# lukehollis/three-mlagents

Hardware: NVIDIA B200
Metric: env_steps_per_sec (higher is better)
Workload: dtype f32+f64

## Files before the change

### profiles/rollout_ab.py

```python
from __future__ import annotations

import argparse
import json
import os
import shutil
import statistics
import subprocess
import sys
import tempfile

import numpy as np

ROOT = os.path.dirname(os.path.dirname(os.path.abspath(__file__)))


def _run(cmd, cwd):
    r = subprocess.run(cmd, cwd=cwd, capture_output=True, text=True)
    if r.returncode != 0:
        raise RuntimeError(f"{' '.join(cmd)} in {cwd} failed ({r.returncode}):\n{r.stdout[-2000:]}\n{r.stderr[-4000:]}")
    return r.stdout


def _bench(tree, steps, dump=None):
    cmd = [sys.executable, "bench.py", "--quick", "--steps", str(steps)] + (["--dump-outputs", dump] if dump else [])
    return json.loads(_run(cmd, tree).strip().splitlines()[-1])


_TASK_TIMER = """
import sys, torch
sys.path.insert(0, '.')
from three_mlagents_b200.vec_env import CudaVecEnv
task, n, T, K = sys.argv[1], 65536, 128, int(sys.argv[2])
env = CudaVecEnv(task, n, seed=1)
obs = torch.empty((T, n, env.obs_dim), device='cuda')
act = torch.empty((T, n), dtype=torch.int32, device='cuda')
rew = torch.empty((T, n), device='cuda')
done = torch.empty((T, n), dtype=torch.uint8, device='cuda')
for _ in range(50):
    env.rollout_random(T, obs, act, rew, done)
e0, e1 = torch.cuda.Event(enable_timing=True), torch.cuda.Event(enable_timing=True)
e0.record()
for _ in range(K):
    env.rollout_random(T, obs, act, rew, done)
e1.record()
torch.cuda.synchronize()
print(e0.elapsed_time(e1) / K * 1e3)
"""


def _time_task(tree, task, steps):
    return float(_run([sys.executable, "-c", _TASK_TIMER, task, str(steps)], tree).strip().splitlines()[-1])


def _summary(runs, base_name="parent"):
    base = statistics.median(runs[base_name])
    return {name: {"us_per_launch": us, "median_us": statistics.median(us), "spread": (max(us) - min(us)) / statistics.median(us),
                   "gain_vs_parent": 1.0 - statistics.median(us) / base} for name, us in runs.items()}


def main():
    ap = argparse.ArgumentParser()
    ap.add_argument("--parent", required=True, help="untracked export of the parent commit")
    ap.add_argument("--rounds", type=int, default=4)
    ap.add_argument("--steps", type=int, default=200)
    ap.add_argument("--tasks", default="gridworld,push", help="tasks also timed through env.rollout_random ('' for none)")
    ap.add_argument("--out", default=os.path.join(ROOT, "profiles", "rollout_blocks_ab_1gpu.json"))
    args = ap.parse_args()
    trees = {"parent": os.path.abspath(args.parent), "new": ROOT}
    q = "name,power.limit,clocks.max.sm"
    card = _run(["nvidia-smi", f"--query-gpu={q}", "--format=csv,noheader", "-i", "0"], ROOT).strip()
    result = {"card": dict(zip(q.split(","), [c.strip() for c in card.split(",")])),
              "bench": f"bench.py --quick --steps {args.steps}", "rounds": args.rounds}
    for tree in trees.values():
        _run([sys.executable, os.path.join(tree, "three-mlagents_b200", "build.py")], tree)
    tmp = tempfile.mkdtemp(prefix="rollout_ab_")
    try:
        for name, tree in trees.items():
            _bench(tree, 50, dump=os.path.join(tmp, name))
        result["dump_equal"] = {f: bool(np.array_equal(np.load(os.path.join(tmp, "parent", f)), np.load(os.path.join(tmp, "new", f))))
                                for f in ("obs.npy", "actions.npy", "rewards.npy", "dones.npy")}
    finally:
        shutil.rmtree(tmp, ignore_errors=True)
    tasks = [t for t in args.tasks.split(",") if t]
    runs = {name: [] for name in trees}
    task_runs = {task: {name: [] for name in trees} for task in tasks}
    for _ in range(args.rounds):
        for name, tree in trees.items():
            runs[name].append(_bench(tree, args.steps)["ms_per_step"] * 1e3)
            print(name, f"{runs[name][-1]:.2f} us", file=sys.stderr, flush=True)
            for task in tasks:
                task_runs[task][name].append(_time_task(tree, task, args.steps))
                print(name, task, f"{task_runs[task][name][-1]:.2f} us", file=sys.stderr, flush=True)
    result["runs"] = _summary(runs)
    if tasks:
        result["rollout_random_65536x128"] = {task: _summary(r) for task, r in task_runs.items()}
    os.makedirs(os.path.dirname(os.path.abspath(args.out)), exist_ok=True)
    with open(args.out, "w") as f:
        json.dump(result, f, indent=1)
    print(json.dumps(result))


if __name__ == "__main__":
    main()
```

### profiles/rollout_sass.py

```python
from __future__ import annotations

import argparse
import os
import re
import subprocess
import sys
import tempfile

ROOT = os.path.dirname(os.path.dirname(os.path.abspath(__file__)))
FLAGS = ["-gencode", "arch=compute_100a,code=sm_100a", "-lineinfo", "-O3", "-std=c++17", "--expt-relaxed-constexpr"]
INS = re.compile(r"^\s+/\*([0-9a-f]{4,})\*/\s+(.*?)\s*;")


def _compile(tree, tmp):
    csrc = os.path.join(tree, "three-mlagents_b200", "csrc")
    cubin = os.path.join(tmp, "env_kernels.cubin")
    nvcc = os.path.join(os.environ.get("CUDA_HOME", "/usr/local/cuda"), "bin", "nvcc")
    r = subprocess.run([nvcc, *FLAGS, "-I", os.path.join(tree, "include"), "-Xptxas", "-v", "-cubin", "-o", cubin,
                        os.path.join(csrc, "env_kernels.cu")], capture_output=True, text=True)
    if r.returncode != 0:
        raise SystemExit(r.stdout + r.stderr)
    return cubin, r.stdout + r.stderr


def _ptxas(log, mangled):
    lines = log.splitlines()
    for n, line in enumerate(lines):
        if f"'{mangled}'" in line and "Compiling entry" in line:
            text = " ".join(lines[n + 1:n + 4])
            num = lambda pat: int(re.search(pat, text).group(1))
            return {"registers": num(r"Used (\d+) registers"), "stack_bytes": num(r"(\d+) bytes stack frame"),
                    "spill_store_bytes": num(r"(\d+) bytes spill stores"), "spill_load_bytes": num(r"(\d+) bytes spill loads")}
    raise SystemExit(f"{mangled}: no ptxas report")


def _sass(cubin, mangled):
    out = subprocess.run(["cuobjdump", "-sass", "-fun", mangled, cubin], capture_output=True, text=True, check=True).stdout
    return [(int(m.group(1), 16), m.group(2)) for m in map(INS.match, out.splitlines()) if m]


def _branch(ins):
    m = re.match(r"(@!?U?P\w+\s+)?BRA(\.U)?\s+(!?U?P\w+,\s*)?(0x[0-9a-f]+)", ins)
    if not m:
        return None
    return int(m.group(4), 16), bool(m.group(1) or m.group(3))


def _loops(code):
    loops = []
    for addr, ins in code:
        b = _branch(ins)
        if b and b[0] <= addr:
            loops.append((b[0], addr))
    return [(h, e) for h, e in loops if not any(h <= h2 and e2 <= e and (h2, e2) != (h, e) for h2, e2 in loops)]


def _shortest(code, head, end):
    body = [(a, ins) for a, ins in code if head <= a <= end]
    index = {a: n for n, (a, _) in enumerate(body)}
    inf = (1 << 30, 0, 0)
    best = [inf] * (len(body) + 1)
    best[0] = (0, 0, 0)
    for n, (a, ins) in enumerate(body):
        if best[n] == inf:
            continue
        c, br, st = best[n]
        here = (c + 1, br + (_branch(ins) is not None), st + ("STG" in ins and ".U8" in ins))
        if a == end:
            best[len(body)] = min(best[len(body)], here)
            continue
        b = _branch(ins)
        nxt = []
        if b is None or b[1]:
            if not re.match(r"(EXIT|RET)", ins):
                nxt.append(n + 1)
        if b and head < b[0] <= end and b[0] in index:
            nxt.append(index[b[0]])
        for m in nxt:
            best[m] = min(best[m], here)
    return best[len(body)]


def main():
    ap = argparse.ArgumentParser()
    ap.add_argument("--tree", default=ROOT, help="repository tree whose env_kernels.cu is compiled")
    ap.add_argument("--tasks", default="Ball3D,GridWorld,Push")
    args = ap.parse_args()
    with tempfile.TemporaryDirectory(prefix="rollout_sass_") as tmp:
        cubin, log = _compile(os.path.abspath(args.tree), tmp)
        for task in args.tasks.split(","):
            name = f"{task}Task"
            mangled = f"_Z19rollout_fast_kernelI{len(name)}{name}Ev7EnvPtrsjmmmiP6float4PiPfPh"
            res = _ptxas(log, mangled)
            code = _sass(cubin, mangled)
            print(f"rollout_fast_kernel<{name}>: {res['registers']} registers, stack {res['stack_bytes']} B, "
                  f"spills {res['spill_store_bytes']} B stored / {res['spill_load_bytes']} B loaded, {len(code) * 16} B of code")
            for head, end in _loops(code):
                ins, br, steps = _shortest(code, head, end)
                if not steps:
                    continue
                per = f", per step {ins / steps:.1f} instructions and {br / steps:.1f} branches"
                print(f"    loop 0x{head:x}-0x{end:x}: {end + 16 - head} B, shortest path {ins} instructions, "
                      f"{br} branches, {steps} steps{per}")


if __name__ == "__main__":
    sys.exit(main())
```

### three-mlagents_b200/csrc/env_handle.cuh

```cuda
#pragma once
#include "common.cuh"

struct tmla_env {
    int task;
    int64_t n;
    uint64_t seed, env_id_base, step_count;
    int device;
    void *buf[4];
    int *err_flag;
    void *d_stage, *h_stage;
    size_t stage_bytes;
    cudaStream_t own_stream;
    int32_t *d_ndone;
    int64_t rec_hint;
    cudaStream_t dev_stream;
    bool dev_dirty;
    cudaEvent_t dev_evt;
    int act_u8;
    void *shadow[4];
    int pend_seq;
    float2 *ep_log;
    int32_t ep_log_cap;
    int32_t *ep_log_count;
    void *rollout_plan;
    void (*rollout_plan_free)(void *);
};

struct DeviceGuard {
    int prev = -1;
    bool switched = false;
    explicit DeviceGuard(int dev) {
        if (cudaGetDevice(&prev) == cudaSuccess && prev != dev) switched = cudaSetDevice(dev) == cudaSuccess;
    }
    ~DeviceGuard() { if (switched) cudaSetDevice(prev); }
};
static inline void mark_device_path(tmla_env *h, cudaStream_t st) { h->dev_stream = st; h->dev_dirty = true; }
```

### three-mlagents_b200/csrc/env_kernels.cu

```cuda
#include <stdarg.h>
#include <stdlib.h>
#include <string.h>
#include <new>
#include <type_traits>
#if defined(__x86_64__)
#include <immintrin.h>
#endif
#include "envs.cuh"
#include "env_handle.cuh"

static int order_after_device_path(tmla_env *h) {
    if (!h->dev_dirty) return TMLA_OK;
    h->dev_dirty = false;
    cudaStreamCaptureStatus cap = cudaStreamCaptureStatusNone;
    if (cudaStreamIsCapturing(h->dev_stream, &cap) != cudaSuccess || cap != cudaStreamCaptureStatusNone ||
        cudaEventRecord(h->dev_evt, h->dev_stream) != cudaSuccess) {
        cudaGetLastError();
        TMLA_CUDA(cudaDeviceSynchronize());
        return TMLA_OK;
    }
    TMLA_CUDA(cudaStreamWaitEvent(h->own_stream, h->dev_evt, 0));
    return TMLA_OK;
}

struct EnvPtrs { void *buf[4]; };

static constexpr int kBlock = 128;

template <int D, int BLOCK, bool STREAMING>
__device__ __forceinline__ void block_store_obs(const float *s_obs, float *dst, int valid_envs) {
    const int total = valid_envs * D;
    if ((reinterpret_cast<uintptr_t>(dst) & 15u) == 0) {
        const int nvec = total >> 2;
        const float4 *s4 = reinterpret_cast<const float4 *>(s_obs);
        float4 *d4 = reinterpret_cast<float4 *>(dst);
        for (int v = threadIdx.x; v < nvec; v += BLOCK) {
            if (STREAMING) st_stream_f4(d4 + v, s4[v]);
            else d4[v] = s4[v];
        }
        for (int e = (nvec << 2) + threadIdx.x; e < total; e += BLOCK) dst[e] = s_obs[e];
    } else {
        for (int e = threadIdx.x; e < total; e += BLOCK) dst[e] = s_obs[e];
    }
}

template <int D>
__device__ __forceinline__ void thread_store_obs(const float *o, float *dst) {
#pragma unroll
    for (int j = 0; j < D; ++j) dst[j] = o[j];
}

template <class Task>
__global__ void __launch_bounds__(kBlock) reset_kernel(EnvPtrs p, int64_t n, uint64_t seed, uint64_t env_base,
                                                       uint64_t k, uint32_t tag, float *obs) {
    __shared__ __align__(16) float s_obs[kBlock * Task::D];
    const int64_t i0 = (int64_t)blockIdx.x * kBlock, i = i0 + threadIdx.x;
    if (i < n) {
        typename Task::State s;
        Task::reset(s, seed, env_base + (uint64_t)i, k, tag);
        Task::store(p.buf, i, s);
        float o[Task::D];
        Task::observe(s, o);
#pragma unroll
        for (int j = 0; j < Task::D; ++j) s_obs[threadIdx.x * Task::D + j] = o[j];
    }
    __syncthreads();
    if (obs) block_store_obs<Task::D, kBlock, false>(s_obs, obs + i0 * Task::D, (int)min((int64_t)kBlock, n - i0));
}

template <class Task>
__global__ void get_state_kernel(EnvPtrs p, int64_t n, typename Task::Wire *aos) {
    const int64_t i = (int64_t)blockIdx.x * blockDim.x + threadIdx.x;
    if (i < n) aos[i] = Task::to_wire(Task::load(p.buf, i));
}
template <class Task>
__global__ void set_state_kernel(EnvPtrs p, int64_t n, const typename Task::Wire *aos) {
    const int64_t i = (int64_t)blockIdx.x * blockDim.x + threadIdx.x;
    if (i < n) Task::store(p.buf, i, Task::from_wire(aos[i]));
}

template <class Task>
__global__ void __launch_bounds__(kBlock)
step_kernel(EnvPtrs p, int64_t n, uint64_t seed, uint64_t env_base, uint64_t step_index,
            const int32_t *__restrict__ actions, float *__restrict__ obs, float *__restrict__ reward,
            uint8_t *__restrict__ done, uint8_t *__restrict__ truncated, float *__restrict__ terminal_obs,
            float *__restrict__ ep_return, int32_t *__restrict__ ep_length, int32_t *n_done, int *err_flag,
            float *__restrict__ compact, int32_t *__restrict__ host_flags, int host_seq, int act_u8,
// ... 105 lines not shown
#pragma unroll
        for (int j = 0; j < D / 2; ++j) s2[j] = make_float2(o[2 * j], o[2 * j + 1]);
    } else {
#pragma unroll
        for (int j = 0; j < D; ++j) stage[threadIdx.x * D + j] = o[j];
    }
}

template <class Task>
__global__ void __launch_bounds__(kRollBlock)
rollout_random_kernel(EnvPtrs p, int64_t n, uint64_t seed, uint64_t env_base, uint64_t step0, int T,
                      float *__restrict__ obs_buf, int32_t *__restrict__ act_buf, float *__restrict__ rew_buf,
                      uint8_t *__restrict__ done_buf) {
    constexpr int D = Task::D, BLOCK = kRollBlock;
    constexpr bool STAGED = (D != 4);
    constexpr int NVEC = BLOCK * D / 4;
    __shared__ __align__(16) float s_obs[STAGED ? 2 * BLOCK * D : 4];
    const int64_t i0 = (int64_t)blockIdx.x * BLOCK, i = i0 + threadIdx.x;
    const bool active = i < n;
    const int valid = (int)min((int64_t)BLOCK, n - i0);
    const uint64_t env_id = env_base + (uint64_t)i;
    const int64_t row_floats = n * D;
    const bool vec_ok = obs_buf && valid == BLOCK && ((reinterpret_cast<uintptr_t>(obs_buf + i0 * D) & 15u) == 0) &&
                        ((row_floats & 3) == 0);
    const typename Task::Consts cst = Task::load_consts();
    typename Task::State s;
    TmlaActionStream as;
    if (active) {
        s = Task::load(p.buf, i);
        as.seek(seed, env_id, step0, Task::A);
    }
    float *orow = obs_buf ? obs_buf + i0 * D : nullptr;
    int64_t off = i;
    for (int t = 0; t < T; ++t) {
        const uint64_t k = step0 + (uint64_t)t;
        float *stage = STAGED ? s_obs + (t & 1) * BLOCK * D : s_obs;
        if (active) {
            float o[D];
            Task::observe(s, o);
            if (STAGED) stage_obs<D>(stage, o);
            else if (obs_buf) {
                float *dst = obs_buf + off * 4;
                if ((reinterpret_cast<uintptr_t>(obs_buf) & 15u) == 0) st_stream_f4(reinterpret_cast<float4 *>(dst), make_float4(o[0], o[1], o[2], o[3]));
                else { dst[0] = o[0]; dst[1] = o[1]; dst[2] = o[2]; dst[3] = o[3]; }
            }
            const int a = as.next(seed, env_id, step0, (uint32_t)t, Task::A);
            float r; bool term, trunc;
            Task::step(cst, s, a, r, term, trunc);
            s.ep_ret = __fadd_rn(s.ep_ret, r);
            const bool d = term || trunc;
            if (act_buf) __stcs(act_buf + off, a);
            if (rew_buf) __stcs(rew_buf + off, r);
            if (done_buf) __stcs(done_buf + off, (uint8_t)(d ? 1 : 0));
            if (d) Task::reset(s, seed, env_id, k + 1, TMLA_TAG_RESET);
        }
        if (STAGED) {
            __syncthreads();
            if (vec_ok) {
                const float4 *s4 = reinterpret_cast<const float4 *>(stage);
                float4 *d4 = reinterpret_cast<float4 *>(orow);
#pragma unroll
                for (int v = 0; v < (NVEC + BLOCK - 1) / BLOCK; ++v) {
                    const int e = v * BLOCK + threadIdx.x;
                    if ((v + 1) * BLOCK <= NVEC || e < NVEC) st_stream_f4(d4 + e, s4[e]);
                }
            } else if (obs_buf) {
                block_store_obs<D, BLOCK, true>(stage, orow, valid);
            }
            if (orow) orow += row_floats;
        }
        off += n;
    }
    if (active) Task::store(p.buf, i, s);
}

#ifndef TMLA_SPARE_EVERY
#define TMLA_SPARE_EVERY 64
#endif
static constexpr int kSpareEvery = TMLA_SPARE_EVERY;
#ifndef TMLA_ROLLOUT_UNROLL
#define TMLA_ROLLOUT_UNROLL 2
#endif
static constexpr int kRollUnroll = TMLA_ROLLOUT_UNROLL;
static_assert(kSpareEvery % 16 == 0 && ((kSpareEvery / 16) & (kSpareEvery / 16 - 1)) == 0, "a power-of-two number of action blocks");
static_assert(16 % kRollUnroll == 0, "the unrolled step loop covers whole action blocks");

template <class Task>
__device__ __noinline__ typename Task::Spare draw_spare(uint64_t seed, uint64_t env_id, uint32_t episode) {
    return Task::draw(seed, env_id, episode, TMLA_TAG_RESET);
}

template <class Task>
__global__ void __launch_bounds__(kRollBlock)
rollout_fast_kernel(EnvPtrs p, uint32_t n, uint64_t seed, uint64_t env_base, uint64_t step0, int T,
                    float4 *__restrict__ obs4, int32_t *__restrict__ act_buf, float *__restrict__ rew_buf,
                    uint8_t *__restrict__ done_buf) {
    constexpr int D = Task::D, BLOCK = kRollBlock, NVEC = BLOCK * D / 4;
    static_assert(Task::A <= 16, "actions are packed as 4-bit digits");
    constexpr bool DIRECT = (D == 6);
    constexpr bool STAGED = (D != 4) && !DIRECT;
    static_assert((BLOCK * D) % 4 == 0, "block rows must be whole float4s");
    __shared__ __align__(16) float s_stage[STAGED ? 2 * BLOCK * D : 4];
    const uint32_t tid = threadIdx.x, i = blockIdx.x * BLOCK + tid;
    const uint64_t env_id = env_base + (uint64_t)i;
    const typename Task::Consts cst = Task::load_consts();
    typename Task::State s = Task::load(p.buf, i);
    float *orow = reinterpret_cast<float *>(obs4) + (size_t)i * D;
    float4 *vrow = obs4 + blockIdx.x * NVEC + tid;
    int32_t *arow = act_buf + i;
    float *rrow = rew_buf + i;
    uint8_t *drow = done_buf + i;
    const uint32_t rowfloats = n * D;
    uint32_t sb = 0;
    [[maybe_unused]] typename Task::Spare sp;
    [[maybe_unused]] bool have_spare = false;
    auto step = [&](uint64_t digits, uint32_t j, uint64_t kb) {
        float o[D];
        Task::observe(s, o);
        if constexpr (STAGED) {
            if constexpr (D % 2 == 0) {
                float2 *s2 = reinterpret_cast<float2 *>(s_stage + sb + tid * D);
#pragma unroll
                for (int q = 0; q < D / 2; ++q) s2[q] = make_float2(o[2 * q], o[2 * q + 1]);
            } else {
#pragma unroll
                for (int q = 0; q < D; ++q) s_stage[sb + tid * D + q] = o[q];
            }
        } else if constexpr (DIRECT) {
            float2 *d2 = reinterpret_cast<float2 *>(orow);
#pragma unroll
            for (int q = 0; q < D / 2; ++q) __stcs(d2 + q, make_float2(o[2 * q], o[2 * q + 1]));
        } else {
            st_stream_f4(reinterpret_cast<float4 *>(orow), make_float4(o[0], o[1], o[2], o[3]));
        }
        const int a = (int)((uint32_t)(digits >> (4 * j)) & 15u);
        float r; bool term, trunc;
        Task::step(cst, s, a, r, term, trunc);
        s.ep_ret = __fadd_rn(s.ep_ret, r);
        const bool d = term || trunc;
        __stcs(arow, a);
        __stcs(rrow, r);
        __stcs(drow, (uint8_t)(d ? 1 : 0));
        if (d) {
            if constexpr (Task::HAS_SPARE) {
                const uint32_t e = Task::next_episode(s);
                if (!have_spare) sp = draw_spare<Task>(seed, env_id, e);
                Task::begin_episode(s, sp, e);
                have_spare = false;
            } else {
                Task::reset(s, seed, env_id, kb + j + 1, TMLA_TAG_RESET);
            }
        }
        if constexpr (STAGED) {
            if constexpr (BLOCK == 32) __syncwarp(); else __syncthreads();
            const float4 *s4 = reinterpret_cast<const float4 *>(s_stage + sb);
#pragma unroll
            for (int v = 0; v < (NVEC + BLOCK - 1) / BLOCK; ++v) {
                const int e = v * BLOCK + tid;
                if ((v + 1) * BLOCK <= NVEC || e < NVEC) st_stream_f4(vrow + v * BLOCK, s4[e]);
            }
            sb ^= BLOCK * D;
            vrow += rowfloats / 4;
        } else {
            orow += rowfloats;
        }
        arow += n; rrow += n; drow += n;
    };
    uint64_t kb = step0 & ~(uint64_t)15;
    uint32_t j = (uint32_t)step0 & 15u;
    uint32_t left = (uint32_t)T;
    for (uint32_t nb = 0; left != 0; ++nb, kb += 16, j = 0) {
        const uint64_t digits = TmlaActionStream::block_digits(seed, env_id, kb >> 4, Task::A);
        if constexpr (Task::HAS_SPARE) {
            if ((nb & (kSpareEvery / 16 - 1)) == 0 && !have_spare) {
                sp = Task::draw(seed, env_id, Task::next_episode(s), TMLA_TAG_RESET);
                have_spare = true;
            }
        }
        if (j == 0 && left >= 16) {
#pragma unroll kRollUnroll
            for (uint32_t q = 0; q < 16; ++q) step(digits, q, kb);
            left -= 16;
        } else {
            const uint32_t je = min(16u, j + left);
            left -= je - j;
#pragma unroll 1
            for (; j < je; ++j) step(digits, j, kb);
        }
    }
    Task::store(p.buf, i, s);
}

template <int A>
__device__ __forceinline__ void categorical(const float *l, bool deterministic, float u, int &action, float &logp) {
    float m = l[0];
#pragma unroll
    for (int j = 1; j < A; ++j) m = fmaxf(m, l[j]);
    float e[A], sum = 0.0f;
#pragma unroll
    for (int j = 0; j < A; ++j) { e[j] = expf(l[j] - m); sum += e[j]; }
    int a = 0;
    if (deterministic) {
#pragma unroll
        for (int j = 1; j < A; ++j) if (l[j] > l[a]) a = j;
    } else {
        const float target = u * sum;
        float c = 0.0f;
        a = A - 1;
        bool found = false;
#pragma unroll
        for (int j = 0; j < A; ++j) {
            c += e[j];
            if (!found && target < c) { a = j; found = true; }
        }
    }
    action = a;
    logp = (l[a] - m) - logf(sum);
}

template <class Task>
__global__ void __launch_bounds__(kBlock)
step_policy_kernel(EnvPtrs p, int64_t n, uint64_t seed, uint64_t env_base, uint64_t step_index,
                   const uint64_t *__restrict__ step_base, const float *__restrict__ logits, int deterministic,
                   int64_t row_index, float *__restrict__ obs_next, int32_t *__restrict__ act, float *__restrict__ logp_out,
                   float *__restrict__ rew, uint8_t *__restrict__ done, int32_t *trunc_count,
                   int32_t *__restrict__ trunc_index, float *__restrict__ trunc_obs, int32_t trunc_capacity,
                   float *ep_stats, float2 *__restrict__ ep_log, int32_t ep_log_cap, int32_t *ep_log_count) {
    constexpr int D = Task::D, A = Task::A;
    __shared__ __align__(16) float s_obs[kBlock * D];
    __shared__ float s_ep[3];
    const int64_t i0 = (int64_t)blockIdx.x * kBlock, i = i0 + threadIdx.x;
    const uint64_t k = step_base ? (*step_base + (uint64_t)row_index) : step_index;
    const unsigned lane = threadIdx.x & 31u, lanes_below = (1u << lane) - 1u;
    if (threadIdx.x < 3) s_ep[threadIdx.x] = 0.0f;
    __syncthreads();
    const bool live = i < n;
    const uint64_t env_id = env_base + (uint64_t)i;
    typename Task::State s;
    float o[D];
    bool d = false, trunc_only = false;
    float ep_r = 0.0f, ep_l = 0.0f;
    if (live) {
        const typename Task::Consts cst = Task::load_consts();
        s = Task::load(p.buf, i);
        float l[A];
#pragma unroll
        for (int j = 0; j < A; ++j) l[j] = logits[i * A + j];
        float u = 0.0f;
        if (!deterministic) u = tmla_u24(tmla_stream_block(seed, env_id, k, TMLA_TAG_SAMPLE, 0).x);
        int a; float lp;
        categorical<A>(l, deterministic != 0, u, a, lp);
        float r; bool term, trunc;
        Task::step(cst, s, a, r, term, trunc);
        s.ep_ret = __fadd_rn(s.ep_ret, r);
        d = term || trunc;
        trunc_only = trunc && !term;
        if (act) act[i] = a;
        if (logp_out) logp_out[i] = lp;
        rew[i] = r;
        done[i] = d ? 1 : 0;
        Task::observe(s, o);
        if (d) { ep_r = s.ep_ret; ep_l = (float)s.steps; }
    }
    if (trunc_count) {
        const unsigned m = __ballot_sync(0xffffffffu, trunc_only);
        if (m) {
            const int leader = __ffs(m) - 1;
            int base = 0;
            if ((int)lane == leader) base = atomicAdd(trunc_count, __popc(m));
            base = __shfl_sync(0xffffffffu, base, leader);
            if (trunc_only) {
// ... 33 lines not shown
#pragma unroll
        for (int j = 0; j < D; ++j) s_obs[threadIdx.x * D + j] = o[j];
    }
    __syncthreads();
    if (ep_stats && threadIdx.x == 0 && s_ep[2] > 0.0f) {
        atomicAdd(ep_stats + 0, s_ep[0]);
        atomicAdd(ep_stats + 1, s_ep[1]);
        atomicAdd(ep_stats + 2, s_ep[2]);
    }
    block_store_obs<D, kBlock, false>(s_obs, obs_next + i0 * D, (int)min((int64_t)kBlock, n - i0));
}

__global__ void counter_add_kernel(uint64_t *c, uint64_t n) { *c += n; }

__global__ void selftest_arith_kernel(unsigned long long *out) {
    const uint32_t tid = blockIdx.x * blockDim.x + threadIdx.x, nth = gridDim.x * blockDim.x;
    unsigned long long bad3 = 0;
    for (uint32_t bits = tid; bits < 0x41000000u; bits += nth) {
        const float x = __uint_as_float(bits);
        bad3 += (__float_as_uint(div3_rn(x)) != __float_as_uint(__fdiv_rn(x, 3.0f)));
    }
    if (bad3) atomicAdd(out + 0, bad3);
    if (tid < 11) {
        const float k = (float)((int)tid - 5);
        if (__float_as_uint(div5_rn(k)) != __float_as_uint(__fdiv_rn(k, 5.0f))) atomicAdd(out + 1, 1ull);
    }
    unsigned long long worst = 0;
    for (uint32_t j = tid; j < (1u << 22); j += nth) {
        const double x = kB3.max_tilt * (2.0 * ((double)j + 0.5) / 4194304.0 - 1.0);
        const long long a = __double_as_longlong(sin_small(x)), b = __double_as_longlong(sin(x));
        const unsigned long long d = (unsigned long long)(a > b ? a - b : b - a);
        worst = d > worst ? d : worst;
    }
    atomicMax(out + 2, worst);
}

#define TASK_SWITCH(task, CALL)                                   \
    switch (task) {                                               \
        case TMLA_BASIC: { using TaskT = BasicTask; CALL; } break;        \
        case TMLA_BALL3D: { using TaskT = Ball3DTask; CALL; } break;      \
        case TMLA_GRIDWORLD: { using TaskT = GridWorldTask; CALL; } break; \
        case TMLA_PUSH: { using TaskT = PushTask; CALL; } break;          \
        case TMLA_WALLJUMP: { using TaskT = WallJumpTask; CALL; } break;  \
        case TMLA_BRICKBREAK: { using TaskT = BrickBreakTask; CALL; } break; \
        case TMLA_BICYCLE: { using TaskT = BicycleTask; CALL; } break;       \
        case TMLA_GLIDER: { using TaskT = GliderTask; CALL; } break;         \
        default: tmla_set_error("unknown task %d", task); return TMLA_EINVAL; \
    }

static EnvPtrs ptrs_of(const tmla_env *h) {
    EnvPtrs p;
    for (int b = 0; b < 4; ++b) p.buf[b] = h->buf[b];
    return p;
}
static inline unsigned grid_for(int64_t n) { return (unsigned)ceil_div64(n, kBlock); }

static const int kObsDim[TMLA_NUM_TASKS] = {BasicTask::D, Ball3DTask::D, GridWorldTask::D, PushTask::D, WallJumpTask::D, BrickBreakTask::D, BicycleTask::D, GliderTask::D};
static const int kNumActions[TMLA_NUM_TASKS] = {BasicTask::A, Ball3DTask::A, GridWorldTask::A, PushTask::A, WallJumpTask::A, BrickBreakTask::A, BicycleTask::A, GliderTask::A};
static const int kMaxSteps[TMLA_NUM_TASKS] = {BasicTask::MAX_STEPS, Ball3DTask::MAX_STEPS, GridWorldTask::MAX_STEPS, PushTask::MAX_STEPS,
                                              WallJumpTask::MAX_STEPS, BrickBreakTask::MAX_STEPS, BicycleTask::MAX_STEPS, GliderTask::MAX_STEPS};
static const int kStateSize[TMLA_NUM_TASKS] = {(int)sizeof(tmla_basic_state), (int)sizeof(tmla_ball3d_state), (int)sizeof(tmla_gridworld_state),
                                               (int)sizeof(tmla_push_state), (int)sizeof(tmla_walljump_state), (int)sizeof(tmla_brickbreak_state),
                                               (int)sizeof(tmla_bicycle_state), (int)sizeof(tmla_glider_state)};

static inline int record_words(int D) { return (3 + D + 3) & ~3; }
struct StageLayout { size_t act, obs, rew, done, trunc, flags, crec, tobs, ret, len, end; };
static StageLayout stage_layout(int64_t n, int D) {
    auto up = [](size_t x) { return (x + 15) & ~(size_t)15; };
    StageLayout L;
    L.act = 0;
    L.obs = up(L.act + 4 * n);
    L.rew = L.obs + 4 * n * D;
    L.done = L.rew + 4 * n;
    L.trunc = L.done + n;
    L.flags = up(L.trunc + n);
    L.crec = L.flags + 16;
    L.tobs = up(L.crec + 4 * n * record_words(D));
    L.ret = L.tobs + 4 * n * D;
    L.len = L.ret + 4 * n;
    L.end = L.len + 4 * n;
    return L;
}


#if defined(__x86_64__)
__attribute__((target("avx2"))) static int64_t stage_actions32_avx2(const int32_t *src, uint8_t *dst, int64_t n, uint64_t *ored, uint32_t *mx) {
    __m256i acc = _mm256_setzero_si256(), vmx = _mm256_setzero_si256();
    const __m256i perm = _mm256_setr_epi32(0, 4, 1, 5, 2, 6, 3, 7);
    int64_t i = 0;
    for (; i + 32 <= n; i += 32) {
        const __m256i a = _mm256_loadu_si256((const __m256i *)(src + i)), b = _mm256_loadu_si256((const __m256i *)(src + i + 8));
        const __m256i c = _mm256_loadu_si256((const __m256i *)(src + i + 16)), d = _mm256_loadu_si256((const __m256i *)(src + i + 24));
        acc = _mm256_or_si256(acc, _mm256_or_si256(_mm256_or_si256(a, b), _mm256_or_si256(c, d)));
        __m256i p = _mm256_packus_epi16(_mm256_packs_epi32(a, b), _mm256_packs_epi32(c, d));
        p = _mm256_permutevar8x32_epi32(p, perm);
        vmx = _mm256_max_epu8(vmx, p);
        _mm256_storeu_si256((__m256i *)(dst + i), p);
    }
    uint64_t t[4]; uint8_t m8[32];
    _mm256_storeu_si256((__m256i *)t, acc); _mm256_storeu_si256((__m256i *)m8, vmx);
    const uint64_t o = t[0] | t[1] | t[2] | t[3];
    *ored |= (o | (o >> 32)) & 0xFFFFFFFFull;
    for (int k = 0; k < 32; ++k) *mx = m8[k] > *mx ? m8[k] : *mx;
    return i;
}
__attribute__((target("avx2"))) static int64_t stage_actions64_avx2(const int64_t *src, uint8_t *dst, int64_t n, uint64_t *ored, uint32_t *mx) {
    __m256i acc = _mm256_setzero_si256(), vmx = _mm256_setzero_si256();
    const __m256i lo = _mm256_setr_epi32(0, 2, 4, 6, 0, 2, 4, 6), perm = _mm256_setr_epi32(0, 4, 1, 5, 2, 6, 3, 7);
    int64_t i = 0;
    for (; i + 32 <= n; i += 32) {
        __m256i w[4];
        for (int k = 0; k < 4; ++k) {
            const __m256i x = _mm256_loadu_si256((const __m256i *)(src + i + 8 * k)), y = _mm256_loadu_si256((const __m256i *)(src + i + 8 * k + 4));
            acc = _mm256_or_si256(acc, _mm256_or_si256(x, y));
            const __m256i xl = _mm256_permutevar8x32_epi32(x, lo), yl = _mm256_permutevar8x32_epi32(y, lo);
            w[k] = _mm256_inserti128_si256(xl, _mm256_castsi256_si128(yl), 1);
        }
        __m256i p = _mm256_packus_epi16(_mm256_packs_epi32(w[0], w[1]), _mm256_packs_epi32(w[2], w[3]));
        p = _mm256_permutevar8x32_epi32(p, perm);
        vmx = _mm256_max_epu8(vmx, p);
        _mm256_storeu_si256((__m256i *)(dst + i), p);
    }
    uint64_t t[4]; uint8_t m8[32];
    _mm256_storeu_si256((__m256i *)t, acc); _mm256_storeu_si256((__m256i *)m8, vmx);
    const uint64_t o = t[0] | t[1] | t[2] | t[3];
    *ored |= (o & ~7ull) ? 0xFFFFFFFFull : (o & 7ull);
    for (int k = 0; k < 32; ++k) *mx = m8[k] > *mx ? m8[k] : *mx;
    return i;
}
#endif

extern "C" {

int tmla_task_from_name(const char *name) {
    if (!name) { tmla_set_error("task name is NULL"); return TMLA_EINVAL; }
    if (!strcmp(name, "basic")) return TMLA_BASIC;
    if (!strcmp(name, "ball3d")) return TMLA_BALL3D;
    if (!strcmp(name, "gridworld")) return TMLA_GRIDWORLD;
    if (!strcmp(name, "push")) return TMLA_PUSH;
    if (!strcmp(name, "walljump")) return TMLA_WALLJUMP;
    if (!strcmp(name, "brickbreak")) return TMLA_BRICKBREAK;
    if (!strcmp(name, "bicycle")) return TMLA_BICYCLE;
    if (!strcmp(name, "glider")) return TMLA_GLIDER;
    tmla_set_error("no CUDA backend for task '%s' (have: basic, ball3d, gridworld, push, walljump, brickbreak, bicycle, glider)", name);
    return TMLA_EINVAL;
}
#define TASK_META(fn, table)                                                                   \
    int fn(int task) {                                                                         \
        if (task < 0 || task >= TMLA_NUM_TASKS) { tmla_set_error(#fn ": unknown task %d", task); return TMLA_EINVAL; } \
        return table[task];                                                                    \
    }
TASK_META(tmla_task_obs_dim, kObsDim)
TASK_META(tmla_task_num_actions, kNumActions)
TASK_META(tmla_task_max_steps, kMaxSteps)
TASK_META(tmla_task_state_size, kStateSize)

int tmla_create(int task, int64_t n_envs, uint64_t seed, uint64_t env_id_base, int device, tmla_env **out) {
    TMLA_REQUIRE(out != nullptr, "out is NULL");
    TMLA_REQUIRE(task >= 0 && task < TMLA_NUM_TASKS, "unknown task");
    TMLA_REQUIRE(n_envs > 0 && n_envs < (int64_t)1 << 31, "n_envs must be in (0, 2^31)");
    int ndev = 0;
    TMLA_CUDA(cudaGetDeviceCount(&ndev));
    TMLA_REQUIRE(device >= 0 && device < ndev, "no such CUDA device (this library has no CPU path)");
    DeviceGuard guard(device);
    tmla_env *h = new (std::nothrow) tmla_env();
    if (!h) { tmla_set_error("out of host memory"); return TMLA_ENOMEM; }
// ... 365 lines not shown

int tmla_step_host(tmla_env *h, const int32_t *actions, float *obs, float *reward, uint8_t *done, uint8_t *truncated,
                   float *terminal_obs, float *ep_return, int32_t *ep_length, int64_t *n_done) {
    TMLA_REQUIRE(h, "handle is NULL");
    TMLA_REQUIRE(actions && obs && reward && done && truncated, "actions/obs/reward/done/truncated must be non-NULL");
    const int64_t n = h->n;
    const int D = kObsDim[h->task];
    const StageLayout L = stage_layout(n, D);
    char *p = (char *)h->h_stage;
    { const int rc = tmla_stage_actions(h, actions, 4); if (rc) return rc; }
    int64_t nd = 0;
    const int rc = step_into_block(h, p + L.obs, &nd);
    if (rc != TMLA_OK && rc != TMLA_EACTION) return rc;
    memcpy(obs, p + L.obs, 4 * n * D);
    memcpy(reward, p + L.rew, 4 * n);
    memcpy(done, p + L.done, n);
    memcpy(truncated, p + L.trunc, n);
    const size_t rec = (size_t)4 * record_words(D);
    for (int64_t s = 0; s < nd; ++s) {
        const float *r = (const float *)(p + L.crec + rec * s);
        int32_t i, l;
        memcpy(&i, r, 4); memcpy(&l, r + 2, 4);
        if (terminal_obs) memcpy(terminal_obs + (size_t)i * D, r + 3, (size_t)4 * D);
        if (ep_return) ep_return[i] = r[1];
        if (ep_length) ep_length[i] = l;
    }
    if (n_done) *n_done = nd;
    return rc;
}

int tmla_reset_host(tmla_env *h, float *obs) {
    TMLA_REQUIRE(h && obs, "handle/obs is NULL");
    DeviceGuard guard(h->device);
    { const int rc = order_after_device_path(h); if (rc) return rc; }
    const size_t bytes = (size_t)4 * h->n * kObsDim[h->task];
    const StageLayout L = stage_layout(h->n, kObsDim[h->task]);
    char *d = (char *)h->d_stage, *p = (char *)h->h_stage;
    int rc = tmla_reset(h, (float *)(d + L.obs), h->own_stream);
    if (rc) return rc;
    TMLA_CUDA(cudaMemcpyAsync(p + L.obs, d + L.obs, bytes, cudaMemcpyDeviceToHost, h->own_stream));
    TMLA_CUDA(cudaStreamSynchronize(h->own_stream));
    if (obs != (float *)(p + L.obs)) memcpy(obs, p + L.obs, bytes);
    return TMLA_OK;
}

int tmla_get_state(tmla_env *h, void *aos, void *stream) {
    TMLA_REQUIRE(h && aos, "handle/aos is NULL");
    DeviceGuard guard(h->device);
    mark_device_path(h, (cudaStream_t)stream);
    TASK_SWITCH(h->task, (get_state_kernel<TaskT><<<grid_for(h->n), kBlock, 0, (cudaStream_t)stream>>>(
                             ptrs_of(h), h->n, (typename TaskT::Wire *)aos)));
    TMLA_LAUNCH_CHECK();
    return TMLA_OK;
}
int tmla_set_state(tmla_env *h, const void *aos, void *stream) {
    TMLA_REQUIRE(h && aos, "handle/aos is NULL");
    DeviceGuard guard(h->device);
    mark_device_path(h, (cudaStream_t)stream);
    TASK_SWITCH(h->task, (set_state_kernel<TaskT><<<grid_for(h->n), kBlock, 0, (cudaStream_t)stream>>>(
                             ptrs_of(h), h->n, (const typename TaskT::Wire *)aos)));
    TMLA_LAUNCH_CHECK();
    return TMLA_OK;
}
int tmla_check_actions(tmla_env *h, void *stream) {
    TMLA_REQUIRE(h, "handle is NULL");
    DeviceGuard guard(h->device);
    int err = 0;
    TMLA_CUDA(cudaMemcpyAsync(&err, h->err_flag, sizeof(int), cudaMemcpyDeviceToHost, (cudaStream_t)stream));
    TMLA_CUDA(cudaStreamSynchronize((cudaStream_t)stream));
    if (err) {
        TMLA_CUDA(cudaMemsetAsync(h->err_flag, 0, sizeof(int), (cudaStream_t)stream));
        tmla_set_error("an action outside [0,%d) was passed to step()", kNumActions[h->task]);
        return TMLA_EACTION;
    }
    return TMLA_OK;
}

int tmla_rollout_random(tmla_env *h, int T, float *obs_buf, int32_t *act_buf, float *rew_buf, uint8_t *done_buf, void *stream) {
    TMLA_REQUIRE(h, "handle is NULL");
    TMLA_REQUIRE(T > 0, "T must be positive");
    DeviceGuard guard(h->device);
    mark_device_path(h, (cudaStream_t)stream);
    const int D = kObsDim[h->task];
    const bool fast = obs_buf && act_buf && rew_buf && done_buf && (h->n % kRollBlock == 0) &&
                      ((reinterpret_cast<uintptr_t>(obs_buf) & 15u) == 0) && ((int64_t)T * h->n * D / 4 < ((int64_t)1 << 31));
    const unsigned grid = (unsigned)ceil_div64(h->n, kRollBlock);
    if (fast) {
        TASK_SWITCH(h->task, (rollout_fast_kernel<TaskT><<<grid, kRollBlock, 0, (cudaStream_t)stream>>>(
                                 ptrs_of(h), (uint32_t)h->n, h->seed, h->env_id_base, h->step_count, T,
                                 reinterpret_cast<float4 *>(obs_buf), act_buf, rew_buf, done_buf)));
    } else {
        TASK_SWITCH(h->task, (rollout_random_kernel<TaskT><<<grid, kRollBlock, 0, (cudaStream_t)stream>>>(
                                 ptrs_of(h), h->n, h->seed, h->env_id_base, h->step_count, T, obs_buf, act_buf, rew_buf, done_buf)));
    }
    TMLA_LAUNCH_CHECK();
    h->step_count += (uint64_t)T;
    return TMLA_OK;
}

int tmla_step_policy(tmla_env *h, const float *logits, int deterministic, int32_t row_index, float *obs_next,
                     int32_t *act, float *logp, float *rew, uint8_t *done, int32_t *trunc_count, int32_t *trunc_index,
                     float *trunc_obs, int32_t trunc_capacity, float *ep_stats, const uint64_t *step_base, void *stream) {
    TMLA_REQUIRE(h, "handle is NULL");
    TMLA_REQUIRE(logits && obs_next && rew && done, "logits/obs_next/rew/done must be non-NULL");
    TMLA_REQUIRE(!trunc_count || (trunc_index && trunc_obs && trunc_capacity > 0), "truncation list is incomplete");
    DeviceGuard guard(h->device);
    mark_device_path(h, (cudaStream_t)stream);
    TASK_SWITCH(h->task, (step_policy_kernel<TaskT><<<grid_for(h->n), kBlock, 0, (cudaStream_t)stream>>>(
                             ptrs_of(h), h->n, h->seed, h->env_id_base, h->step_count, step_base, logits, deterministic,
                             (int64_t)row_index, obs_next, act, logp, rew, done, trunc_count, trunc_index, trunc_obs,
                             trunc_capacity, ep_stats, h->ep_log, h->ep_log_cap, h->ep_log_count)));
    TMLA_LAUNCH_CHECK();
    if (!step_base) h->step_count += 1;
    return TMLA_OK;
}

int tmla_selftest_arith(uint64_t *out3, void *stream) {
    TMLA_REQUIRE(out3, "out3 is NULL");
    TMLA_CUDA(cudaMemsetAsync(out3, 0, 3 * sizeof(uint64_t), (cudaStream_t)stream));
    selftest_arith_kernel<<<148 * 8, 256, 0, (cudaStream_t)stream>>>((unsigned long long *)out3);
    TMLA_LAUNCH_CHECK();
    return TMLA_OK;
}

int tmla_counter_add(uint64_t *counter, uint64_t n, void *stream) {
    TMLA_REQUIRE(counter, "counter is NULL");
    counter_add_kernel<<<1, 1, 0, (cudaStream_t)stream>>>(counter, n);
    TMLA_LAUNCH_CHECK();
    return TMLA_OK;
}

}
```

Measured before the change: 150.1 billion.

## Stage rollout outputs in shared memory and write them with TMA bulk tensor stores

For tasks with small observation rows, the rollout kernel now writes obs, action, reward and done values for a chunk of four steps into a double-buffered shared-memory tile. The block leader then issues 2D cp.async.bulk.tensor stores with an L2 evict_first hint. Tensor maps are encoded on the host and cached per buffer set and T. This replaces many per-thread streaming global stores, including byte-wide done stores, with bulk transfers. In exchange it adds proxy fences, wait_group stalls on the leader, warp syncs, more shared memory, and a host-side map re-encode whenever the buffers change.

```diff
diff --git a/profiles/rollout_ab.py b/profiles/rollout_ab.py
--- a/profiles/rollout_ab.py
+++ b/profiles/rollout_ab.py
@@ -64,7 +64,7 @@
     ap.add_argument("--rounds", type=int, default=4)
     ap.add_argument("--steps", type=int, default=200)
     ap.add_argument("--tasks", default="gridworld,push", help="tasks also timed through env.rollout_random ('' for none)")
-    ap.add_argument("--out", default=os.path.join(ROOT, "profiles", "rollout_blocks_ab_1gpu.json"))
+    ap.add_argument("--out", default=os.path.join(ROOT, "profiles", "rollout_tma_ab_1gpu.json"))
     args = ap.parse_args()
     trees = {"parent": os.path.abspath(args.parent), "new": ROOT}
     q = "name,power.limit,clocks.max.sm"
diff --git a/profiles/rollout_sass.py b/profiles/rollout_sass.py
--- a/profiles/rollout_sass.py
+++ b/profiles/rollout_sass.py
@@ -58,14 +58,17 @@
 def _shortest(code, head, end):
     body = [(a, ins) for a, ins in code if head <= a <= end]
     index = {a: n for n, (a, _) in enumerate(body)}
-    inf = (1 << 30, 0, 0)
+    inf = (1 << 30, 0, 0, ())
     best = [inf] * (len(body) + 1)
-    best[0] = (0, 0, 0)
+    best[0] = (0, 0, 0, ())
     for n, (a, ins) in enumerate(body):
         if best[n] == inf:
             continue
-        c, br, st = best[n]
-        here = (c + 1, br + (_branch(ins) is not None), st + ("STG" in ins and ".U8" in ins))
+        c, br, st, stores = best[n]
+        op = ins.split()[0] if not ins.startswith("@") else ins.split()[1]
+        kind = op.split(".")[0]
+        here = (c + 1, br + (_branch(ins) is not None), st + (kind in ("STG", "STS") and ".U8" in op),
+                stores + ((kind,) if kind in ("STG", "STS", "UTMASTG") else ()))
         if a == end:
             best[len(body)] = min(best[len(body)], here)
             continue
@@ -74,7 +77,8 @@
         if b is None or b[1]:
             if not re.match(r"(EXIT|RET)", ins):
                 nxt.append(n + 1)
-        if b and head < b[0] <= end and b[0] in index:
+        leader_only = b and b[0] > a and any(op.startswith(("UTMASTG", "DEPBAR")) for x, op in body[n + 1:] if x < b[0])
+        if b and head < b[0] <= end and b[0] in index and not leader_only:
             nxt.append(index[b[0]])
         for m in nxt:
             best[m] = min(best[m], here)
@@ -90,18 +94,21 @@
         cubin, log = _compile(os.path.abspath(args.tree), tmp)
         for task in args.tasks.split(","):
             name = f"{task}Task"
-            mangled = f"_Z19rollout_fast_kernelI{len(name)}{name}Ev7EnvPtrsjmmmiP6float4PiPfPh"
+            mangled = re.search(rf"'(_Z19rollout_fast_kernelI{len(name)}{name}Ev\w+)'", log).group(1)
             res = _ptxas(log, mangled)
             code = _sass(cubin, mangled)
             print(f"rollout_fast_kernel<{name}>: {res['registers']} registers, stack {res['stack_bytes']} B, "
                   f"spills {res['spill_store_bytes']} B stored / {res['spill_load_bytes']} B loaded, {len(code) * 16} B of code")
             for head, end in _loops(code):
-                ins, br, steps = _shortest(code, head, end)
+                ins, br, steps, stores = _shortest(code, head, end)
                 if not steps:
                     continue
                 per = f", per step {ins / steps:.1f} instructions and {br / steps:.1f} branches"
+                kinds = ", ".join(f"{stores.count(k)} {k}" for k in ("STG", "STS", "UTMASTG"))
                 print(f"    loop 0x{head:x}-0x{end:x}: {end + 16 - head} B, shortest path {ins} instructions, "
-                      f"{br} branches, {steps} steps{per}")
+                      f"{br} branches, {steps} steps{per}; stores on the path: {kinds}")
+            tma = sum(ins.startswith("UTMASTG") or " UTMASTG" in ins for _, ins in code)
+            print(f"    UTMASTG in the kernel: {tma}")
 
 
 if __name__ == "__main__":
diff --git a/three-mlagents_b200/csrc/env_handle.cuh b/three-mlagents_b200/csrc/env_handle.cuh
--- a/three-mlagents_b200/csrc/env_handle.cuh
+++ b/three-mlagents_b200/csrc/env_handle.cuh
@@ -1,5 +1,8 @@
 #pragma once
+#include <cuda.h>
 #include "common.cuh"
+
+struct RolloutMaps { CUtensorMap obs, act, rew, done; };
 
 struct tmla_env {
     int task;
@@ -24,6 +27,9 @@
     int32_t *ep_log_count;
     void *rollout_plan;
     void (*rollout_plan_free)(void *);
+    RolloutMaps rollout_maps;
+    const void *rollout_map_bufs[4];
+    int rollout_map_T;
 };
 
 struct DeviceGuard {
diff --git a/three-mlagents_b200/csrc/env_kernels.cu b/three-mlagents_b200/csrc/env_kernels.cu
--- a/three-mlagents_b200/csrc/env_kernels.cu
+++ b/three-mlagents_b200/csrc/env_kernels.cu
@@ -3,6 +3,7 @@
 #include <string.h>
 #include <new>
 #include <type_traits>
+#include <cudaTypedefs.h>
 #if defined(__x86_64__)
 #include <immintrin.h>
 #endif
@@ -274,8 +275,33 @@
 #define TMLA_ROLLOUT_UNROLL 2
 #endif
 static constexpr int kRollUnroll = TMLA_ROLLOUT_UNROLL;
+static constexpr int kRollChunk = 4;
 static_assert(kSpareEvery % 16 == 0 && ((kSpareEvery / 16) & (kSpareEvery / 16 - 1)) == 0, "a power-of-two number of action blocks");
 static_assert(16 % kRollUnroll == 0, "the unrolled step loop covers whole action blocks");
+static_assert(16 % kRollChunk == 0, "an action block holds whole chunks");
+
+__host__ __device__ constexpr bool rollout_uses_tma(int D) { return kRollBlock * D <= 256; }
+
+template <int D>
+struct RollChunk {
+    static constexpr uint32_t up(uint32_t x) { return (x + 127u) & ~127u; }
+    static constexpr uint32_t OBS_ROW = kRollBlock * D * 4, ROW = kRollBlock * 4, DONE_ROW = kRollBlock;
+    static constexpr uint32_t OBS = 0, ACT = up(kRollChunk * OBS_ROW), REW = ACT + up(kRollChunk * ROW),
+                              DONE = REW + up(kRollChunk * ROW), BYTES = up(DONE + kRollChunk * DONE_ROW);
+};
+
+__device__ __forceinline__ void sts_f32(uint32_t a, float x) { asm volatile("st.shared.f32 [%0], %1;" ::"r"(a), "f"(x)); }
+__device__ __forceinline__ void sts_f32x2(uint32_t a, float x, float y) { asm volatile("st.shared.v2.f32 [%0], {%1, %2};" ::"r"(a), "f"(x), "f"(y)); }
+__device__ __forceinline__ void sts_f32x4(uint32_t a, float x, float y, float z, float w) {
+    asm volatile("st.shared.v4.f32 [%0], {%1, %2, %3, %4};" ::"r"(a), "f"(x), "f"(y), "f"(z), "f"(w));
+}
+__device__ __forceinline__ void sts_s32(uint32_t a, int32_t x) { asm volatile("st.shared.s32 [%0], %1;" ::"r"(a), "r"(x)); }
+__device__ __forceinline__ void sts_u8(uint32_t a, uint16_t x) { asm volatile("st.shared.u8 [%0], %1;" ::"r"(a), "h"(x)); }
+
+__device__ __forceinline__ void tma_store_rows(const CUtensorMap *map, uint32_t src, int32_t x, int32_t y, uint64_t policy) {
+    asm volatile("cp.async.bulk.tensor.2d.global.shared::cta.bulk_group.L2::cache_hint [%0, {%1, %2}], [%3], %4;"
+                 ::"l"(reinterpret_cast<uint64_t>(map)), "r"(x), "r"(y), "r"(src), "l"(policy) : "memory");
+}
 
 template <class Task>
 __device__ __noinline__ typename Task::Spare draw_spare(uint64_t seed, uint64_t env_id, uint32_t episode) {
@@ -285,54 +311,67 @@
 template <class Task>
 __global__ void __launch_bounds__(kRollBlock)
 rollout_fast_kernel(EnvPtrs p, uint32_t n, uint64_t seed, uint64_t env_base, uint64_t step0, int T,
-                    float4 *__restrict__ obs4, int32_t *__restrict__ act_buf, float *__restrict__ rew_buf,
-                    uint8_t *__restrict__ done_buf) {
-    constexpr int D = Task::D, BLOCK = kRollBlock, NVEC = BLOCK * D / 4;
+                    const __grid_constant__ RolloutMaps maps, float4 *__restrict__ obs4, int32_t *__restrict__ act_buf,
+                    float *__restrict__ rew_buf, uint8_t *__restrict__ done_buf) {
+    constexpr int D = Task::D, BLOCK = kRollBlock, NVEC = BLOCK * D / 4, C = kRollChunk;
+    constexpr bool TMA = rollout_uses_tma(D);
+    using L = RollChunk<D>;
     static_assert(Task::A <= 16, "actions are packed as 4-bit digits");
-    constexpr bool DIRECT = (D == 6);
-    constexpr bool STAGED = (D != 4) && !DIRECT;
     static_assert((BLOCK * D) % 4 == 0, "block rows must be whole float4s");
-    __shared__ __align__(16) float s_stage[STAGED ? 2 * BLOCK * D : 4];
+    __shared__ __align__(128) unsigned char s_chunk[TMA ? 2 * L::BYTES : 16];
+    __shared__ __align__(16) float s_stage[TMA ? 4 : 2 * BLOCK * D];
     const uint32_t tid = threadIdx.x, i = blockIdx.x * BLOCK + tid;
     const uint64_t env_id = env_base + (uint64_t)i;
     const typename Task::Consts cst = Task::load_consts();
     typename Task::State s = Task::load(p.buf, i);
-    float *orow = reinterpret_cast<float *>(obs4) + (size_t)i * D;
+    const uint32_t s_base = (uint32_t)__cvta_generic_to_shared(s_chunk);
+    const uint32_t s_obs = s_base + L::OBS + tid * (D * 4), s_word = s_base + tid * 4, s_done = s_base + L::DONE + tid;
     float4 *vrow = obs4 + blockIdx.x * NVEC + tid;
     int32_t *arow = act_buf + i;
     float *rrow = rew_buf + i;
     uint8_t *drow = done_buf + i;
     const uint32_t rowfloats = n * D;
     uint32_t sb = 0;
+    [[maybe_unused]] uint64_t evict_first = 0;
+    if constexpr (TMA) asm("createpolicy.fractional.L2::evict_first.b64 %0, 1.0;" : "=l"(evict_first));
     [[maybe_unused]] typename Task::Spare sp;
     [[maybe_unused]] bool have_spare = false;
-    auto step = [&](uint64_t digits, uint32_t j, uint64_t kb) {
+    auto step = [&](int a, uint64_t k, uint32_t buf, uint32_t slot) {
         float o[D];
         Task::observe(s, o);
-        if constexpr (STAGED) {
-            if constexpr (D % 2 == 0) {
-                float2 *s2 = reinterpret_cast<float2 *>(s_stage + sb + tid * D);
-#pragma unroll
-                for (int q = 0; q < D / 2; ++q) s2[q] = make_float2(o[2 * q], o[2 * q + 1]);
+        if constexpr (TMA) {
+            const uint32_t so = s_obs + buf + slot * L::OBS_ROW;
+            if constexpr (D % 4 == 0) {
+#pragma unroll
+                for (int q = 0; q < D / 4; ++q) sts_f32x4(so + 16 * q, o[4 * q], o[4 * q + 1], o[4 * q + 2], o[4 * q + 3]);
+            } else if constexpr (D % 2 == 0) {
+#pragma unroll
+                for (int q = 0; q < D / 2; ++q) sts_f32x2(so + 8 * q, o[2 * q], o[2 * q + 1]);
             } else {
 #pragma unroll
-                for (int q = 0; q < D; ++q) s_stage[sb + tid * D + q] = o[q];
+                for (int q = 0; q < D; ++q) sts_f32(so + 4 * q, o[q]);
             }
-        } else if constexpr (DIRECT) {
-            float2 *d2 = reinterpret_cast<float2 *>(orow);
-#pragma unroll
-            for (int q = 0; q < D / 2; ++q) __stcs(d2 + q, make_float2(o[2 * q], o[2 * q + 1]));
+        } else if constexpr (D % 2 == 0) {
+            float2 *s2 = reinterpret_cast<float2 *>(s_stage + sb + tid * D);
+#pragma unroll
+            for (int q = 0; q < D / 2; ++q) s2[q] = make_float2(o[2 * q], o[2 * q + 1]);
         } else {
-            st_stream_f4(reinterpret_cast<float4 *>(orow), make_float4(o[0], o[1], o[2], o[3]));
-        }
-        const int a = (int)((uint32_t)(digits >> (4 * j)) & 15u);
+#pragma unroll
+            for (int q = 0; q < D; ++q) s_stage[sb + tid * D + q] = o[q];
+        }
         float r; bool term, trunc;
         Task::step(cst, s, a, r, term, trunc);
         s.ep_ret = __fadd_rn(s.ep_ret, r);
         const bool d = term || trunc;
-        __stcs(arow, a);
-        __stcs(rrow, r);
-        __stcs(drow, (uint8_t)(d ? 1 : 0));
+        if constexpr (TMA) {
+            sts_s32(s_word + buf + L::ACT + slot * L::ROW, a);
+            sts_f32(s_word + buf + L::REW + slot * L::ROW, r);
+            sts_u8(s_done + buf + slot * L::DONE_ROW, d ? 1 : 0);
+        } else {
+            __stcs(arow, a);
+            __stcs(rrow, r);
+            __stcs(drow, (uint8_t)(d ? 1 : 0));
+        }
         if (d) {
             if constexpr (Task::HAS_SPARE) {
                 const uint32_t e = Task::next_episode(s);
@@ -340,10 +379,10 @@
                 Task::begin_episode(s, sp, e);
                 have_spare = false;
             } else {
-                Task::reset(s, seed, env_id, kb + j + 1, TMLA_TAG_RESET);
+                Task::reset(s, seed, env_id, k + 1, TMLA_TAG_RESET);
             }
         }
-        if constexpr (STAGED) {
+        if constexpr (!TMA) {
             if constexpr (BLOCK == 32) __syncwarp(); else __syncthreads();
             const float4 *s4 = reinterpret_cast<const float4 *>(s_stage + sb);
 #pragma unroll
@@ -353,14 +392,27 @@
             }
             sb ^= BLOCK * D;
             vrow += rowfloats / 4;
-        } else {
-            orow += rowfloats;
-        }
-        arow += n; rrow += n; drow += n;
+            arow += n; rrow += n; drow += n;
+        }
+    };
+    const bool leader = tid == 0;
+    auto flush = [&](uint32_t buf, int32_t y) {
+        asm volatile("fence.proxy.async.shared::cta;" ::: "memory");
+        if (leader) asm volatile("cp.async.bulk.wait_group.read 0;" ::: "memory");
+        __syncwarp();
+        if (leader) {
+            const uint32_t sa = s_base + buf;
+            tma_store_rows(&maps.obs, sa + L::OBS, (int32_t)(blockIdx.x * BLOCK * D), y, evict_first);
+            tma_store_rows(&maps.act, sa + L::ACT, (int32_t)(blockIdx.x * BLOCK), y, evict_first);
+            tma_store_rows(&maps.rew, sa + L::REW, (int32_t)(blockIdx.x * BLOCK), y, evict_first);
+            tma_store_rows(&maps.done, sa + L::DONE, (int32_t)(blockIdx.x * BLOCK), y, evict_first);
+            asm volatile("cp.async.bulk.commit_group;" ::: "memory");
+        }
     };
     uint64_t kb = step0 & ~(uint64_t)15;
     uint32_t j = (uint32_t)step0 & 15u;
     uint32_t left = (uint32_t)T;
+    uint32_t t = 0;
     for (uint32_t nb = 0; left != 0; ++nb, kb += 16, j = 0) {
         const uint64_t digits = TmlaActionStream::block_digits(seed, env_id, kb >> 4, Task::A);
         if constexpr (Task::HAS_SPARE) {
@@ -369,16 +421,37 @@
                 have_spare = true;
             }
         }
-        if (j == 0 && left >= 16) {
+        if (j == 0 && left >= 16 && (!TMA || t % C == 0)) {
+            if constexpr (TMA) {
+                uint32_t buf = ((t / C) & 1) * L::BYTES;
+#pragma unroll 1
+                for (uint32_t c = 0; c < 16; c += C, buf ^= L::BYTES) {
+                    const uint32_t dc = (uint32_t)(digits >> (4 * c));
+#pragma unroll
+                    for (uint32_t q = 0; q < C; ++q) step((int)((dc >> (4 * q)) & 15u), kb + c + q, buf, q);
+                    flush(buf, (int32_t)(t + c));
+                }
+            } else {
 #pragma unroll kRollUnroll
-            for (uint32_t q = 0; q < 16; ++q) step(digits, q, kb);
+                for (uint32_t q = 0; q < 16; ++q) step((int)((uint32_t)(digits >> (4 * q)) & 15u), kb + q, 0, 0);
+            }
             left -= 16;
+            t += 16;
         } else {
             const uint32_t je = min(16u, j + left);
             left -= je - j;
 #pragma unroll 1
-            for (; j < je; ++j) step(digits, j, kb);
-        }
+            for (; j < je; ++j, ++t) {
+                const uint32_t buf = ((t / C) & 1) * L::BYTES;
+                step((int)((uint32_t)(digits >> (4 * j)) & 15u), kb + j, buf, t % C);
+                if constexpr (TMA) {
+                    if (t % C == C - 1 || (left == 0 && j + 1 == je)) flush(buf, (int32_t)(t & ~(uint32_t)(C - 1)));
+                }
+            }
+        }
+    }
+    if constexpr (TMA) {
+        if (leader) asm volatile("cp.async.bulk.wait_group 0;" ::: "memory");
     }
     Task::store(p.buf, i, s);
 }
@@ -578,6 +651,41 @@
     return L;
 }
 
+
+static int rollout_maps(tmla_env *h, int T, float *obs, int32_t *act, float *rew, uint8_t *done) {
+    const void *bufs[4] = {obs, act, rew, done};
+    if (h->rollout_map_T == T && !memcmp(h->rollout_map_bufs, bufs, sizeof(bufs))) return TMLA_OK;
+    static const PFN_cuTensorMapEncodeTiled_v12000 encode = [] {
+        void *fn = nullptr;
+        cudaDriverEntryPointQueryResult q;
+        if (cudaGetDriverEntryPointByVersion("cuTensorMapEncodeTiled", &fn, 12000, cudaEnableDefault, &q) != cudaSuccess ||
+            q != cudaDriverEntryPointSuccess) {
+            cudaGetLastError();
+            fn = nullptr;
+        }
+        return reinterpret_cast<PFN_cuTensorMapEncodeTiled_v12000>(fn);
+    }();
+    if (!encode) { tmla_set_error("tmla_rollout_random: the driver has no cuTensorMapEncodeTiled"); return TMLA_ECUDA; }
+    h->rollout_map_T = 0;
+    const uint64_t n = (uint64_t)h->n, D = (uint64_t)kObsDim[h->task];
+    struct { CUtensorMap *map; CUtensorMapDataType type; void *base; uint64_t cols, elem; uint32_t box_cols; } rows[4] = {
+        {&h->rollout_maps.obs, CU_TENSOR_MAP_DATA_TYPE_FLOAT32, obs, n * D, 4, (uint32_t)(kRollBlock * D)},
+        {&h->rollout_maps.act, CU_TENSOR_MAP_DATA_TYPE_INT32, act, n, 4, kRollBlock},
+        {&h->rollout_maps.rew, CU_TENSOR_MAP_DATA_TYPE_FLOAT32, rew, n, 4, kRollBlock},
+        {&h->rollout_maps.done, CU_TENSOR_MAP_DATA_TYPE_UINT8, done, n, 1, kRollBlock}};
+    for (const auto &r : rows) {
+        const cuuint64_t dims[2] = {r.cols, (cuuint64_t)T}, strides[1] = {r.cols * r.elem};
+        const cuuint32_t box[2] = {r.box_cols, (cuuint32_t)kRollChunk}, estride[2] = {1, 1};
+        const CUresult e = encode(r.map, r.type, 2, r.base, dims, strides, box, estride, CU_TENSOR_MAP_INTERLEAVE_NONE,
+                                  CU_TENSOR_MAP_SWIZZLE_NONE, CU_TENSOR_MAP_L2_PROMOTION_NONE, CU_TENSOR_MAP_FLOAT_OOB_FILL_NONE);
+        if (e != CUDA_SUCCESS) { tmla_set_error("tmla_rollout_random: cuTensorMapEncodeTiled failed (%d)", (int)e); return TMLA_ECUDA; }
+    }
+    TASK_SWITCH(h->task, TMLA_CUDA(cudaFuncSetAttribute(rollout_fast_kernel<TaskT>, cudaFuncAttributePreferredSharedMemoryCarveout,
+                                                        (int)cudaSharedmemCarveoutMaxShared)));
+    memcpy(h->rollout_map_bufs, bufs, sizeof(bufs));
+    h->rollout_map_T = T;
+    return TMLA_OK;
+}
 
 #if defined(__x86_64__)
 __attribute__((target("avx2"))) static int64_t stage_actions32_avx2(const int32_t *src, uint8_t *dst, int64_t n, uint64_t *ored, uint32_t *mx) {
@@ -1109,12 +1217,22 @@
     DeviceGuard guard(h->device);
     mark_device_path(h, (cudaStream_t)stream);
     const int D = kObsDim[h->task];
-    const bool fast = obs_buf && act_buf && rew_buf && done_buf && (h->n % kRollBlock == 0) &&
-                      ((reinterpret_cast<uintptr_t>(obs_buf) & 15u) == 0) && ((int64_t)T * h->n * D / 4 < ((int64_t)1 << 31));
     const unsigned grid = (unsigned)ceil_div64(h->n, kRollBlock);
+    const bool full = obs_buf && act_buf && rew_buf && done_buf && (h->n % kRollBlock == 0);
+    bool fast;
+    if (rollout_uses_tma(D)) {
+        fast = full && (((reinterpret_cast<uintptr_t>(obs_buf) | reinterpret_cast<uintptr_t>(act_buf) | reinterpret_cast<uintptr_t>(rew_buf) |
+                          reinterpret_cast<uintptr_t>(done_buf)) & 15u) == 0) && h->n * D < ((int64_t)1 << 31);
+        if (fast) {
+            const int rc = rollout_maps(h, T, obs_buf, act_buf, rew_buf, done_buf);
+            if (rc) return rc;
+        }
+    } else {
+        fast = full && ((reinterpret_cast<uintptr_t>(obs_buf) & 15u) == 0) && ((int64_t)T * h->n * D / 4 < ((int64_t)1 << 31));
+    }
     if (fast) {
         TASK_SWITCH(h->task, (rollout_fast_kernel<TaskT><<<grid, kRollBlock, 0, (cudaStream_t)stream>>>(
-                                 ptrs_of(h), (uint32_t)h->n, h->seed, h->env_id_base, h->step_count, T,
+                                 ptrs_of(h), (uint32_t)h->n, h->seed, h->env_id_base, h->step_count, T, h->rollout_maps,
                                  reinterpret_cast<float4 *>(obs_buf), act_buf, rew_buf, done_buf)));
     } else {
         TASK_SWITCH(h->task, (rollout_random_kernel<TaskT><<<grid, kRollBlock, 0, (cudaStream_t)stream>>>(
```

Result: faster. 153.2 billion, median of 6 (+2.1%).
